# andrewadare/SLAM.jl

Measured on AMD Instinct MI355X. Metric: EKF updates/sec @ 10k landmarks, higher is better.
Workload: dtype f32; 1 GPU; EKF-SLAM observation step (associate+update; no new features arise), N=10000 landmarks (n=20003), nz=64 obs/step, gates 4.0/25.0, cholesky form, state resident in HBM; landmarks=10000, form=cholesky, parallelism=single GPU

## Files before the change

slam.jl_amd/csrc/common.h:

```cpp
#pragma once

#include <hip/hip_runtime.h>
#include <stdint.h>
#include <stdio.h>
#include <string.h>
#include <vector>

#include "../../include/slamhip.h"
#include "../../include/slamhip_diag.h"

#define SLAM_PI 3.14159265358979323846

void slam_set_error(const char* fmt, ...);

#define HIP_TRY(expr)                                                                  \
    do {                                                                               \
        hipError_t _e = (expr);                                                        \
        if (_e != hipSuccess) {                                                        \
            slam_set_error("%s failed: %s (%s:%d)", #expr, hipGetErrorString(_e),     \
                           __FILE__, __LINE__);                                        \
            return (_e == hipErrorOutOfMemory) ? SLAM_E_NOMEM : SLAM_E_HIP;            \
        }                                                                              \
    } while (0)

#define ARG_CHECK(cond, msg)                                                           \
    do {                                                                               \
        if (!(cond)) {                                                                 \
            slam_set_error("bad argument: %s", msg);                                   \
            return SLAM_E_BADARG;                                                      \
        }                                                                              \
    } while (0)

void slam_roctx_push(const char* name);
void slam_roctx_pop(void);
struct SlamRange {
    explicit SlamRange(const char* name) { slam_roctx_push(name); }
    ~SlamRange() { slam_roctx_pop(); }
    SlamRange(const SlamRange&) = delete;
    SlamRange& operator=(const SlamRange&) = delete;
};
#define SLAM_RANGE() SlamRange slam_range_scope_(__func__)

#define SLAM_TILE 128
#define SLAM_KPAD 32

static inline int round_up(int a, int b) { return (a + b - 1) / b * b; }

#ifdef SLAMHIP_EXPERIMENTS
#include <stdlib.h>
static inline int slam_exp_env(const char* name, int dflt) {
    const char* v = getenv(name);
    return v ? atoi(v) : dflt;
}
constexpr int SLAM_XFLAGS_MASK = ~0;
#else
static inline int slam_exp_env(const char*, int dflt) { return dflt; }
constexpr int SLAM_XFLAGS_MASK = 4 | 8 | 16 | 32 | 64 | 128 | 512;
#endif

struct TimingPair {
    hipEvent_t a, b;
    int kid;
};

struct slam_ekf {
    int dtype;
    int device;
    int num_cus;
    int maxN;
    int N;
    int ncap;
    int ld;
    int npad;
    size_t esz;
    void* x;
    void* P;
    void* Pside;
    hipStream_t stream;
    double* PHtS;
    hipEvent_t stage_ev;
    int stage_pending;

    int kcap;
    double* PHt;
    double* Kd;
    void* W1;
    void* W2;
    void* Wimg;
    double* Cmat;
    double* Smat;
    double* Mwork;
    double* gvec;
    double* obsbuf;
    int32_t* idfbuf;
    int ocap;
    double* h_obs;
    int32_t* h_idf;
    int32_t* h_assoc;
    int32_t* d_assoc;
    double* h_obs_dev;
    int32_t* h_assoc_dev;
    double* znbuf;
    int32_t* d_count;
    int32_t* h_flag;
    int32_t* h_flag_dev;
    int32_t obs_seq;

    int2* tiles;
    int tiles_T, tiles_len, tiles_cap;
    int tilesB_off, tilesB_len;
    int tilesH_off, tilesH_len;
    unsigned* dd_claim;
    int tiles_xlen[8];
    int diag_off, diag_len, diag_xlen[8];

    double* d_pmax;
    int pmax_valid;

    int gate_mode;
    int gate_last;
    void* grid_meta;
    int32_t* grid_cells;
    void* grid_items;
    int grid_force;
    int grid_upd;
    int grid_live;
    int grid_n_seen;

    double* gate_part;
    int gate_blocks_cap;

    double* d_small;
    double* h_small;
    int32_t* d_status;
    int32_t* h_status;

    int xflags;
    int debug_flags;
    void* dd_prof;
    int factor_blocked;
    int debug_stamps;
    int async_updates;
    int deferred;
    int pending_status;

    int timing;
    std::vector<TimingPair> pairs;
    std::vector<TimingPair> free_pairs;
    double t_ms[SLAM_K_COUNT];
    double t_sq[SLAM_K_COUNT];
    double t_min[SLAM_K_COUNT];
    int64_t t_n[SLAM_K_COUNT];
};

struct KTimer {
    slam_ekf* h;
    TimingPair p;
    bool on;
    hipStream_t s;
    KTimer(slam_ekf* h_, int kid, hipStream_t stream = nullptr);
    ~KTimer();
};

int launch_ellipses(slam_ekf* h, double* d_out);
int launch_block_gather(slam_ekf* h, int r0, int c0, int nr, int nc, int diag, void* d_out);
int launch_pack(slam_ekf* h, const void* d_src, int lds, int n, int cf, int ncols);
int launch_unpack(slam_ekf* h, void* d_dst, int ldd, int n, int cf, int ncols);
int launch_side_rebuild(slam_ekf* h);
int launch_compact(slam_ekf* h, const int32_t* keep_host, int n_new, int f0);
int launch_find_duplicates(slam_ekf* h, double gate, int32_t* pairs_out, int cap, int* count);
int launch_merge_update(slam_ekf* h, const int32_t* keep, const int32_t* gone, int cnt, const double Rc[4]);
int launch_copy_floor(slam_ekf* h, int reps, double out[2]);
int launch_predict(slam_ekf* h, double v, double g, double w, const double Q[4], double dt);
int launch_augment(slam_ekf* h, int nn, const double R[4], const double* zn_dev);
int launch_gate(slam_ekf* h, int nz, const double R[4], double gate1, double gate2, const double* z_host, bool compact);
constexpr int SLAM_GRID_SLOTS = 64;
int gate_kernels_init();
int gate_info(slam_ekf* h, int64_t out[8]);
unsigned long long* grid_drift_slot(slam_ekf* h);
int ensure_pmax(slam_ekf* h);
int launch_nis(slam_ekf* h, const double z1[2], int j, const double R[4]);
int launch_obs_model(slam_ekf* h, int j);
int launch_update(slam_ekf* h, int m, const double R[4], int form, bool device_count);
int ensure_update_workspace(slam_ekf* h, int m);
int ensure_obs_capacity(slam_ekf* h, int nobs);
```

slam.jl_amd/csrc/ekf_syrk.hip:

```cpp
#include <algorithm>
#include <stdlib.h>

#include "common.h"
#include <type_traits>
#include "device_math.h"

namespace {

typedef float f32x16 __attribute__((ext_vector_type(16)));
typedef float f32x4 __attribute__((ext_vector_type(4)));

constexpr int TILE = SLAM_TILE;
constexpr int KC = 32;
constexpr int LDSP = KC + 4;

__device__ __forceinline__ void wave_lds_fence() {
    __builtin_amdgcn_fence(__ATOMIC_RELEASE, "wavefront");
    __builtin_amdgcn_wave_barrier();
    __builtin_amdgcn_fence(__ATOMIC_ACQUIRE, "wavefront");
}

typedef unsigned u32x4 __attribute__((ext_vector_type(4)));

struct DdCtxP {
// ... 192 lines not shown
    for (int rb = 0; rb < 2; ++rb)
#pragma unroll
        for (int r = 0; r < 16; ++r) {
            const int soff = ((32 * c.wc + 8 * (r >> 2) + (r & 3)) * TILE + 64 * c.wr + 32 * rb) * 4;
            pold[rb][r] = __uint_as_float(__builtin_amdgcn_raw_buffer_load_b32(rs, voff, soff, AUX));
        }
}

template <int AUX = 2>
__device__ __forceinline__ void store_p_mfma(const DdCtx& c, int R0, int C0, const float (&pold)[2][16], f32x16 (&acc)[2]) {
    const auto rs = tile_rsrc(c, R0, C0);
    const int voff = (4 * c.lh * TILE + c.l31) * 4;
    const bool adj = R0 == C0 + TILE;
#pragma unroll
    for (int rb = 0; rb < 2; ++rb)
#pragma unroll
        for (int r = 0; r < 16; ++r) {
            const int soff = ((32 * c.wc + 8 * (r >> 2) + (r & 3)) * TILE + 64 * c.wr + 32 * rb) * 4;
            const float v = pold[rb][r] - acc[rb][r];
            __builtin_amdgcn_raw_buffer_store_b32(__float_as_uint(v), rs, voff, soff, AUX);
            if (rb == 0 && r == 15 && adj && c.wr == 0 && c.wc == 3 && c.lh == 1 && c.l31 == 0) c.side[(size_t)c.side_n + ((C0 + TILE - 4) >> 1)] = v;
            acc[rb][r] = 0.0f;
        }
}

template <int NCH, int POFF = 2>
__device__ __forceinline__ void dd_stream(DdCtx& c, const int2* __restrict__ list, int L, int nper, int& slot, smem_t& smem,
                                          f32x4 (&gx)[2], f32x4 (&gy)[2]) {
    auto fetch = [&](int sl) { return sl < L ? list[sl] : make_int2(-1, -1); };
    constexpr int PCH = NCH - POFF > 0 ? NCH - POFF : 0;
    int2 tile = fetch(slot);
    int2 next = fetch(slot + nper);
    f32x16 acc[2];
#pragma unroll
    for (int rb = 0; rb < 2; ++rb)
#pragma unroll
        for (int r = 0; r < 16; ++r) acc[rb][r] = 0.0f;
    float pold[2][16];
    Frag f0;
    const int last_steps = (c.kp - (NCH - 1) * KC <= 16) ? 2 : 4;
    fill_lds(c, smem, 0, gx, gy);
    __syncthreads();
    request_chunk(c, tile, 1, gx, gy);
    int base = 0;
    for (;;) {
        const bool next_off = next.x >= 0 && next.x != next.y;
#pragma unroll
        for (int ch = 0; ch < NCH; ++ch) {
            const int pb = (base + ch) & 1;
            if (ch == PCH) load_p_mfma(c, tile.x * TILE, tile.y * TILE, pold);
            if (ch < NCH - 1) {
#pragma unroll
                for (int st = 0; st < 4; ++st) {
                    read_frag(c, smem, pb, 8 * st, f0);
                    mfma_step(c, f0, acc);
                }
                fill_lds(c, smem, pb ^ 1, gx, gy);
                __syncthreads();
                if (ch + 2 < NCH) request_chunk(c, tile, ch + 2, gx, gy);
                else if (next.x >= 0) request_chunk(c, next, 0, gx, gy);
            } else {
                for (int st = 0; st < last_steps; ++st) {
                    read_frag(c, smem, pb, 8 * st, f0);
                    mfma_step(c, f0, acc);
                }
                if (next_off) fill_lds(c, smem, pb ^ 1, gx, gy);
                __syncthreads();
                if (next_off) request_chunk(c, next, 1, gx, gy);
                store_p_mfma(c, tile.x * TILE, tile.y * TILE, pold, acc);
            }
        }
        slot += nper;
        if (!next_off) return;
        tile = next;
        next = fetch(slot + nper);
        base = (base + NCH) & 1;
    }
}

typedef __bf16 bf16x8 __attribute__((ext_vector_type(8)));
typedef __bf16 bf16x2 __attribute__((ext_vector_type(2)));
typedef float f32x2 __attribute__((ext_vector_type(2)));
typedef unsigned u32x2 __attribute__((ext_vector_type(2)));
constexpr int KB = 16;
constexpr int BROW = 48;
constexpr int BARR = TILE * BROW;

__device__ __forceinline__ int stage_row(int tid) {
    return (tid >> 6) * 16 + ((tid >> 5) & 1) * 8 + ((tid >> 4) & 1) + 2 * ((tid >> 2) & 3);
}

__device__ __forceinline__ void request_chunk_b(const DdCtx& c, int2 t, int chunk, f32x4& gx, f32x4& gy) {
    const auto rx = __builtin_amdgcn_make_buffer_rsrc(const_cast<float*>(c.X), (short)0, c.ld * c.pitch * 4, 0x00020000);
    const auto ry = __builtin_amdgcn_make_buffer_rsrc(const_cast<float*>(c.Y), (short)0, c.ld * c.pitch * 4, 0x00020000);
    const int tid = threadIdx.x;
    const int voff = (stage_row(tid) * c.pitch + 4 * (tid & 3)) * 4;
    gx = __builtin_bit_cast(f32x4, __builtin_amdgcn_raw_buffer_load_b128(rx, voff, (t.x * TILE * c.pitch + chunk * KB) * 4, 0));
    gy = __builtin_bit_cast(f32x4, __builtin_amdgcn_raw_buffer_load_b128(ry, voff, (t.y * TILE * c.pitch + chunk * KB) * 4, 0));
}

__device__ __forceinline__ void split2(float v0, float v1, unsigned& h, unsigned& m, unsigned& l) {
    const f32x2 v = {v0, v1};
    h = __builtin_bit_cast(unsigned, __builtin_convertvector(v, bf16x2));
    const f32x2 r1 = {v0 - __uint_as_float(h << 16), v1 - __uint_as_float(h & 0xffff0000u)};
    m = __builtin_bit_cast(unsigned, __builtin_convertvector(r1, bf16x2));
    const f32x2 r2 = {r1.x - __uint_as_float(m << 16), r1.y - __uint_as_float(m & 0xffff0000u)};
    l = __builtin_bit_cast(unsigned, __builtin_convertvector(r2, bf16x2));
}

__device__ __forceinline__ void fill_lds_b(const DdCtx& c, char* sm, int buf, const f32x4& gx, const f32x4& gy) {
    const int tid = threadIdx.x;
    char* base = sm + buf * (6 * BARR) + stage_row(tid) * BROW + (tid & 3) * 8;
#pragma unroll
    for (int pnl = 0; pnl < 2; ++pnl) {
        const f32x4 g = pnl ? gy : gx;
        unsigned h0, m0, l0, h1, m1, l1;
        split2(g.x, g.y, h0, m0, l0);
        split2(g.z, g.w, h1, m1, l1);
        *reinterpret_cast<u32x2*>(base + (3 * pnl + 0) * BARR) = u32x2{h0, h1};
        *reinterpret_cast<u32x2*>(base + (3 * pnl + 1) * BARR) = u32x2{m0, m1};
        *reinterpret_cast<u32x2*>(base + (3 * pnl + 2) * BARR) = u32x2{l0, l1};
    }
}

__device__ __forceinline__ void mfma_chunk_b(const DdCtx& c, const char* sm, int buf, f32x16 (&acc)[2]) {
    const char* base = sm + buf * (6 * BARR) + c.l31 * BROW + c.lh * 16;
    bf16x8 a[3];
#pragma unroll
    for (int sp = 0; sp < 3; ++sp) a[sp] = *reinterpret_cast<const bf16x8*>(base + (3 + sp) * BARR + (32 * c.wc) * BROW);
#pragma unroll
    for (int rb = 0; rb < 2; ++rb) {
        bf16x8 b[3];
#pragma unroll
        for (int sp = 0; sp < 3; ++sp) b[sp] = *reinterpret_cast<const bf16x8*>(base + sp * BARR + (64 * c.wr + 32 * rb) * BROW);
        __builtin_amdgcn_s_setprio(3);
        acc[rb] = __builtin_amdgcn_mfma_f32_32x32x16_bf16(a[1], b[1], acc[rb], 0, 0, 0);
        acc[rb] = __builtin_amdgcn_mfma_f32_32x32x16_bf16(a[0], b[2], acc[rb], 0, 0, 0);
        acc[rb] = __builtin_amdgcn_mfma_f32_32x32x16_bf16(a[2], b[0], acc[rb], 0, 0, 0);
        acc[rb] = __builtin_amdgcn_mfma_f32_32x32x16_bf16(a[0], b[1], acc[rb], 0, 0, 0);
        acc[rb] = __builtin_amdgcn_mfma_f32_32x32x16_bf16(a[1], b[0], acc[rb], 0, 0, 0);
        acc[rb] = __builtin_amdgcn_mfma_f32_32x32x16_bf16(a[0], b[0], acc[rb], 0, 0, 0);
        __builtin_amdgcn_s_setprio(0);
    }
}

constexpr int IMG_ARR = TILE * 32;
constexpr int IMG_CHUNK = 3 * IMG_ARR;
typedef unsigned u32x4b __attribute__((ext_vector_type(4)));

__device__ __forceinline__ void request_chunk_p(const DdCtx& c, int2 t, int chunk, u32x4b (&g)[3]) {
    const auto rs = __builtin_amdgcn_make_buffer_rsrc(const_cast<char*>(c.img), (short)0, 0x7fffffff, 0x00020000);
    const int tid = threadIdx.x;
    const int sx = (t.x * c.img_nch + chunk) * IMG_CHUNK, sy = (t.y * c.img_nch + chunk) * IMG_CHUNK;
    g[0] = __builtin_amdgcn_raw_buffer_load_b128(rs, tid * 16, sx, 0);
    g[1] = tid < 256 ? __builtin_amdgcn_raw_buffer_load_b128(rs, (tid + 512) * 16, sx, 0)
                     : __builtin_amdgcn_raw_buffer_load_b128(rs, (tid - 256) * 16, sy, 0);
    g[2] = __builtin_amdgcn_raw_buffer_load_b128(rs, (tid + 256) * 16, sy, 0);
}

__device__ __forceinline__ void fill_lds_p(char* sm, int buf, const u32x4b (&g)[3]) {
    char* base = sm + buf * (2 * IMG_CHUNK) + threadIdx.x * 16;
#pragma unroll
    for (int j = 0; j < 3; ++j) *reinterpret_cast<u32x4b*>(base + j * 8192) = g[j];
}

__device__ __forceinline__ void mfma_chunk_p(const DdCtx& c, const char* sm, int buf, f32x16 (&acc)[2], bool negate = false) {
    const char* base = sm + buf * (2 * IMG_CHUNK) + c.l31 * 32 + ((c.lh ^ (c.l31 >> 3)) & 1) * 16;
    bf16x8 a[3];
#pragma unroll
    for (int sp = 0; sp < 3; ++sp) a[sp] = *reinterpret_cast<const bf16x8*>(base + IMG_CHUNK + sp * IMG_ARR + (32 * c.wc) * 32);
    bf16x8 b[3];
#pragma unroll
    for (int rb = 0; rb < 2; ++rb) {
#pragma unroll
        for (int sp = 0; sp < 3; ++sp) b[sp] = *reinterpret_cast<const bf16x8*>(base + sp * IMG_ARR + (64 * c.wr + 32 * rb) * 32);
        __builtin_amdgcn_s_setprio(3);
        acc[rb] = __builtin_amdgcn_mfma_f32_32x32x16_bf16(a[1], b[1], acc[rb], 0, 0, 0);
        acc[rb] = __builtin_amdgcn_mfma_f32_32x32x16_bf16(a[0], b[2], acc[rb], 0, 0, 0);
        acc[rb] = __builtin_amdgcn_mfma_f32_32x32x16_bf16(a[2], b[0], acc[rb], 0, 0, 0);
        acc[rb] = __builtin_amdgcn_mfma_f32_32x32x16_bf16(a[0], b[1], acc[rb], 0, 0, 0);
        acc[rb] = __builtin_amdgcn_mfma_f32_32x32x16_bf16(a[1], b[0], acc[rb], 0, 0, 0);
        acc[rb] = __builtin_amdgcn_mfma_f32_32x32x16_bf16(a[0], b[0], acc[rb], 0, 0, 0);
        __builtin_amdgcn_s_setprio(0);
    }
}

constexpr int CLAIM_OFF = 2 * 2 * IMG_CHUNK;
typedef __attribute__((address_space(3))) unsigned lds_u32_t;
__device__ __forceinline__ void lds_store_u32(char* p, unsigned v) { *(volatile lds_u32_t*)p = v; }
__device__ __forceinline__ unsigned lds_load_u32(const char* p) { return *(const volatile lds_u32_t*)p; }
#ifndef DD_PCH0
#define DD_PCH0 0
#endif
#ifndef DD_DMA_PCH8
#define DD_DMA_PCH8 2
#endif
#ifndef DD_POFF8
#define DD_POFF8 (7 + DD_PCH0)
#endif

template <int NCH, int POFF, bool WRAP = false, bool DYN = false>
__device__ __forceinline__ void dd_stream_p(DdCtx& c, const int2* __restrict__ list, int L, int nper, int& slot, char* sm,
                                            unsigned* __restrict__ ctr = nullptr) {
    auto fetch = [&](int sl) { return sl < L ? list[sl] : make_int2(-1, -1); };
    auto request_chunk_p = [&](const DdCtx& cc, int2 t, int chunk, u32x4b (&gg)[3]) { ::request_chunk_p(cc, t, WRAP ? (chunk & 7) : chunk, gg); };
    constexpr int PCH = NCH - POFF > 0 ? NCH - POFF : 0;
    static_assert(!DYN || NCH >= 4, "the claimed position is read after chunk 1 and used at chunk NCH - 2");
    int2 tile = fetch(slot);
    int2 next = DYN ? make_int2(-1, -1) : fetch(slot + nper);
    int next_slot = slot + nper;
    unsigned claimed = 0;
    f32x16 acc[2];
#pragma unroll
    for (int rb = 0; rb < 2; ++rb)
#pragma unroll
        for (int r = 0; r < 16; ++r) acc[rb][r] = 0.0f;
    float pold[2][16];
    u32x4b g[3];
    request_chunk_p(c, tile, 0, g);
    fill_lds_p(sm, 0, g);
    __syncthreads();
    request_chunk_p(c, tile, 1, g);
    int base = 0;
    for (;;) {
        bool next_off = next.x >= 0 && next.x != next.y;
#pragma unroll
        for (int ch = 0; ch < NCH; ++ch) {
            const int pb = (base + ch) & 1;
            if (ch == PCH) load_p_mfma(c, tile.x * TILE, tile.y * TILE, pold);
            mfma_chunk_p(c, sm, pb, acc, WRAP && ch >= 8);
            if (DYN && ch == 1 && threadIdx.x == 0) lds_store_u32(sm + CLAIM_OFF, claimed);
            if (ch < NCH - 1) {
                fill_lds_p(sm, pb ^ 1, g);
                __syncthreads();
                if (DYN && ch == 0 && threadIdx.x == 0)
                    claimed = __hip_atomic_fetch_add(ctr, 1u, __ATOMIC_RELAXED, __HIP_MEMORY_SCOPE_AGENT);
                if (DYN && ch == 1) {
                    next_slot = nper + __builtin_amdgcn_readfirstlane((int)lds_load_u32(sm + CLAIM_OFF));
                    next = fetch(next_slot);
                    next_off = next.x >= 0 && next.x != next.y;
                }
                if (ch + 2 < NCH) request_chunk_p(c, tile, ch + 2, g);
                else if (next_off) request_chunk_p(c, next, 0, g);
            } else {
                if (next_off) fill_lds_p(sm, pb ^ 1, g);
                __syncthreads();
                if (next_off) request_chunk_p(c, next, 1, g);
                store_p_mfma(c, tile.x * TILE, tile.y * TILE, pold, acc);
            }
        }
        slot = DYN ? next_slot : slot + nper;
        if (!next_off) return;
        tile = next;
        if (!DYN) next = fetch(slot + nper);
        base = (base + NCH) & 1;
    }
}


constexpr int DMA_BUF = 2 * IMG_CHUNK;
typedef __attribute__((address_space(3))) void lds_void_t;

__device__ __forceinline__ void dma_chunk(const DdCtx& c, int2 t, int chunk, char* sm, int buf, int wave) {
    const auto rs = __builtin_amdgcn_make_buffer_rsrc(const_cast<char*>(c.img), (short)0, 0x7fffffff, 0x00020000);
    const int sx = (t.x * c.img_nch + chunk) * IMG_CHUNK + wave * 1024, sy = (t.y * c.img_nch + chunk) * IMG_CHUNK + wave * 1024;
    const int lane16 = (threadIdx.x & 63) * 16;
    char* dst = sm + buf * DMA_BUF + wave * 1024;
    __builtin_amdgcn_raw_ptr_buffer_load_lds(rs, (lds_void_t*)dst, 16, lane16, sx, 0, 0);
    __builtin_amdgcn_raw_ptr_buffer_load_lds(rs, (lds_void_t*)(dst + 8192), 16, lane16, wave < 4 ? sx + 8192 : sy - 4096, 0, 0);
    __builtin_amdgcn_raw_ptr_buffer_load_lds(rs, (lds_void_t*)(dst + 16384), 16, lane16, sy + 4096, 0, 0);
}
__device__ __forceinline__ unsigned lds_addr(const char* p) { return (unsigned)(unsigned long long)(const lds_void_t*)p; }
__device__ __forceinline__ void asm_lds_store_u32(char* p, unsigned v) {
    asm volatile("ds_write_b32 %0, %1" ::"v"(lds_addr(p)), "v"(v) : "memory");
}
__device__ __forceinline__ unsigned asm_lds_load_u32(const char* p) {
    unsigned v;
    asm volatile("ds_read_b32 %0, %1\n\ts_waitcnt lgkmcnt(0)" : "=v"(v) : "v"(lds_addr(p)) : "memory");
    return v;
}
template <int I, int N, typename F>
__device__ __forceinline__ void static_for(F&& f) {
    if constexpr (I < N) {
        f(std::integral_constant<int, I>{});
        static_for<I + 1, N>(f);
    }
}
template <int N>
__device__ __forceinline__ void wait_vm() { asm volatile("s_waitcnt vmcnt(%0)" ::"n"(N) : "memory"); }
__device__ __forceinline__ void bare_barrier() { asm volatile("s_waitcnt lgkmcnt(0)\n\ts_barrier" ::: "memory"); }

struct DdFrags { bf16x8 a[3], b[3], b1[3]; };
__device__ __forceinline__ void read_frags_d(const DdCtx& c, const char* sm, int buf, DdFrags& f) {
    const unsigned base = lds_addr(sm) + buf * DMA_BUF + c.l31 * 32 + ((c.lh ^ (c.l31 >> 3)) & 1) * 16;
    const unsigned ya = base + IMG_CHUNK + (32 * c.wc) * 32, xa = base + (64 * c.wr) * 32;
    asm volatile(
        "ds_read_b128 %0, %9\n\tds_read_b128 %1, %9 offset:4096\n\tds_read_b128 %2, %9 offset:8192\n\t"
        "ds_read_b128 %3, %10\n\tds_read_b128 %4, %10 offset:4096\n\tds_read_b128 %5, %10 offset:8192\n\t"
        "ds_read_b128 %6, %10 offset:1024\n\tds_read_b128 %7, %10 offset:5120\n\tds_read_b128 %8, %10 offset:9216\n\t"
        "s_waitcnt lgkmcnt(0)"
        : "=&v"(f.a[0]), "=&v"(f.a[1]), "=&v"(f.a[2]), "=&v"(f.b[0]), "=&v"(f.b[1]), "=&v"(f.b[2]), "=&v"(f.b1[0]), "=&v"(f.b1[1]), "=&v"(f.b1[2])
        : "v"(ya), "v"(xa)
        : "memory");
}
__device__ __forceinline__ void mfma_frags_d(const DdFrags& f, f32x16 (&acc)[2]) {
#pragma unroll
    for (int rb = 0; rb < 2; ++rb) {
        __builtin_amdgcn_s_setprio(3);
        acc[rb] = __builtin_amdgcn_mfma_f32_32x32x16_bf16(f.a[1], rb ? f.b1[1] : f.b[1], acc[rb], 0, 0, 0);
        acc[rb] = __builtin_amdgcn_mfma_f32_32x32x16_bf16(f.a[0], rb ? f.b1[2] : f.b[2], acc[rb], 0, 0, 0);
        acc[rb] = __builtin_amdgcn_mfma_f32_32x32x16_bf16(f.a[2], rb ? f.b1[0] : f.b[0], acc[rb], 0, 0, 0);
        acc[rb] = __builtin_amdgcn_mfma_f32_32x32x16_bf16(f.a[0], rb ? f.b1[1] : f.b[1], acc[rb], 0, 0, 0);
        acc[rb] = __builtin_amdgcn_mfma_f32_32x32x16_bf16(f.a[1], rb ? f.b1[0] : f.b[0], acc[rb], 0, 0, 0);
        acc[rb] = __builtin_amdgcn_mfma_f32_32x32x16_bf16(f.a[0], rb ? f.b1[0] : f.b[0], acc[rb], 0, 0, 0);
        __builtin_amdgcn_s_setprio(0);
    }
}

template <int NCH, int PCH>
__device__ __forceinline__ void dd_stream_dma(DdCtx& c, const int2* __restrict__ list, int L, int nper, int& slot, char* sm,
                                              unsigned* __restrict__ ctr, int wave, char* cw) {
    static_assert(NCH >= 5 && PCH >= 2 && PCH <= NCH - 2, "");
    constexpr int RD = NCH - 3;
    auto fetch = [&](int sl) { return sl < L ? list[sl] : make_int2(-1, -1); };
    int2 tile = fetch(slot);
    int2 next = make_int2(-1, -1);
    int next_slot = slot + nper;
    unsigned claimed = 0;
    f32x16 acc[2];
#pragma unroll
    for (int rb = 0; rb < 2; ++rb)
#pragma unroll
        for (int r = 0; r < 16; ++r) acc[rb][r] = 0.0f;
    float pold[2][16];
    dma_chunk(c, tile, 0, sm, 0, wave);
    dma_chunk(c, tile, 1, sm, 1, wave);
    dma_chunk(c, tile, 2, sm, 2, wave);
    wait_vm<6>();
    bare_barrier();
    int base = 0;
    bool first = true;
    for (;;) {
        bool next_off = false;
        static_for<0, NCH>([&](auto CH) {
            constexpr int ch = decltype(CH)::value;
            const int buf = (base + ch) % 3;
            __builtin_amdgcn_sched_barrier(0);
            if (ch == PCH) load_p_mfma(c, tile.x * TILE, tile.y * TILE, pold);
            DdFrags fr;
            read_frags_d(c, sm, buf, fr);
            mfma_frags_d(fr, acc);
            if (ch == RD && threadIdx.x == 0) asm_lds_store_u32(cw, claimed);
            constexpr int PL = (ch == PCH || ch == PCH + 1) ? 32 : 0;
            if (ch <= 1) {
                if (first) wait_vm<3>();
                else wait_vm<35>();
            } else if (ch + 2 < NCH || next_off) wait_vm<3 + PL>();
            else wait_vm<PL>();
            bare_barrier();
            if (ch == 0 && threadIdx.x == 0) claimed = __hip_atomic_fetch_add(ctr, 1u, __ATOMIC_RELAXED, __HIP_MEMORY_SCOPE_AGENT);
            if (ch == RD) {
                next_slot = nper + __builtin_amdgcn_readfirstlane((int)asm_lds_load_u32(cw));
                next = fetch(next_slot);
                next_off = next.x >= 0 && next.x != next.y;
            }
            if (ch + 3 < NCH) dma_chunk(c, tile, ch + 3, sm, buf, wave);
            else if (next_off) dma_chunk(c, next, ch + 3 - NCH, sm, buf, wave);
            __builtin_amdgcn_sched_barrier(0);
            if (ch == NCH - 1) store_p_mfma(c, tile.x * TILE, tile.y * TILE, pold, acc);
        });
        slot = next_slot;
        if (!next_off) break;
        tile = next;
        base = (base + NCH) % 3;
        first = false;
    }
    wait_vm<0>();
}

template <int NCH, int POFF, int AUXL = 2, int AUXS = 2>
__device__ __forceinline__ void dd_stream_b(DdCtx& c, const int2* __restrict__ list, int L, int nper, int& slot, char* sm,
                                            f32x4& gx, f32x4& gy) {
    auto fetch = [&](int sl) { return sl < L ? list[sl] : make_int2(-1, -1); };
    constexpr int PCH = NCH - POFF > 0 ? NCH - POFF : 0;
    int2 tile = fetch(slot);
    int2 next = fetch(slot + nper);
    f32x16 acc[2];
#pragma unroll
    for (int rb = 0; rb < 2; ++rb)
#pragma unroll
        for (int r = 0; r < 16; ++r) acc[rb][r] = 0.0f;
    float pold[2][16];
    fill_lds_b(c, sm, 0, gx, gy);
    __syncthreads();
    request_chunk_b(c, tile, 1, gx, gy);
    int base = 0;
    for (;;) {
        const bool next_off = next.x >= 0 && next.x != next.y;
#pragma unroll
        for (int ch = 0; ch < NCH; ++ch) {
            const int pb = (base + ch) & 1;
            if (ch == PCH) load_p_mfma<AUXL>(c, tile.x * TILE, tile.y * TILE, pold);
            mfma_chunk_b(c, sm, pb, acc);
            if (ch < NCH - 1) {
                fill_lds_b(c, sm, pb ^ 1, gx, gy);
                __syncthreads();
                if (ch + 2 < NCH) request_chunk_b(c, tile, ch + 2, gx, gy);
                else if (next_off) request_chunk_b(c, next, 0, gx, gy);
            } else {
                if (next_off) fill_lds_b(c, sm, pb ^ 1, gx, gy);
                __syncthreads();
                if (next_off) request_chunk_b(c, next, 1, gx, gy);
                store_p_mfma<AUXS>(c, tile.x * TILE, tile.y * TILE, pold, acc);
            }
        }
        slot += nper;
        if (!next_off) return;
        tile = next;
        next = fetch(slot + nper);
        base = (base + NCH) & 1;
    }
}

template <int STREAM = 0, int POFF = 2, bool BF = false>
__global__ __launch_bounds__(NTHREADS) __attribute__((amdgpu_waves_per_eu(4, 4))) void downdate_f32_mfma(float* __restrict__ P, int ld, int n,
                                                                 const float* __restrict__ X, const float* __restrict__ Y,
                                                                 int pitch, int kp, const int2* __restrict__ tiles, int L,
                                                                 const int32_t* __restrict__ status, int xflags,
                                                                 const int32_t* __restrict__ dcount, int joseph,
                                                                 const char* __restrict__ img, int img_nch,
                                                                 unsigned* __restrict__ claim,
                                                                 float* __restrict__ side, int side_n) {
    if (status[0] != 0) return;
    if (dcount) {
        const int k = 2 * dcount[0];
        kp = joseph ? 2 * ((k + SLAM_KPAD - 1) / SLAM_KPAD * SLAM_KPAD) : (k + 15) / 16 * 16;
        if (kp == 0) return;
    }
    __shared__ __attribute__((aligned(16))) float smem[2][2][TILE][LDSP];
    __shared__ unsigned dma_claim_word[4];
    const int tid = threadIdx.x;
    const int lane = tid & 63;
    const int wave = __builtin_amdgcn_readfirstlane(tid >> 6);
    DdCtx c;
    c.side = side; c.side_n = side_n;
    c.P = P; c.X = X; c.Y = Y; c.ld = ld; c.pitch = pitch; c.kp = kp; c.xflags = xflags;
    c.img = img; c.img_nch = img_nch;
    c.nchunks = (kp + KC - 1) / KC;
    c.wr = wave & 1;
    c.wc = wave >> 1;
    c.l31 = lane & 31;
    c.lh = lane >> 5;
    c.q = lane & 7;
    c.cl = lane >> 3;
    c.srow = tid >> 3;
    c.sc4 = tid & 7;
    const int xcd = blockIdx.x & 7;
    const int rk = blockIdx.x >> 3;
    const int nper = gridDim.x >> 3;
    if (nper < L && rk >= (nper >> 1) && !claim) __builtin_amdgcn_s_sleep(127);
    const int2* list = tiles + (size_t)xcd * L;
    float* sD = &smem[0][0][0][0] + wave * (2 * 32 * SP);
    float* sV = sD + 32 * SP;
    (void)n;

    int slot = rk;
    int2 tile = slot < L ? list[slot] : make_int2(-1, -1);
    if (tile.x < 0) return;
    f32x4 gx[2], gy[2];
    if (BF && claim && img && kp >= 5 * KB && kp <= 8 * KB && !joseph) {
        char* sm = reinterpret_cast<char*>(&smem[0][0][0][0]);
        unsigned* ctr = claim + 16 * xcd;
        if (tile.x != tile.y && !(c.xflags & 512)) {
            static_assert(sizeof(smem) == 3 * DMA_BUF, "three 24 KB chunk buffers");
            char* cw = reinterpret_cast<char*>(&dma_claim_word[0]);
            switch (kp / KB) {
                case 8: dd_stream_dma<8, DD_DMA_PCH8>(c, list, L, nper, slot, sm, ctr, wave, cw); break;
                case 7: dd_stream_dma<7, 2>(c, list, L, nper, slot, sm, ctr, wave, cw); break;
                case 6: dd_stream_dma<6, 2>(c, list, L, nper, slot, sm, ctr, wave, cw); break;
                default: dd_stream_dma<5, 2>(c, list, L, nper, slot, sm, ctr, wave, cw); break;
            }
        } else
        if (tile.x != tile.y) {
            switch (kp / KB) {
                case 8: dd_stream_p<8, DD_POFF8, false, true>(c, list, L, nper, slot, sm, ctr); break;
                case 7: dd_stream_p<7, 6 + DD_PCH0, false, true>(c, list, L, nper, slot, sm, ctr); break;
                case 6: dd_stream_p<6, 5 + DD_PCH0, false, true>(c, list, L, nper, slot, sm, ctr); break;
                default: dd_stream_p<5, 4 + DD_PCH0, false, true>(c, list, L, nper, slot, sm, ctr); break;
            }
        }
        while (slot < L) {
            tile = list[slot];
            if (tile.x < 0) break;
            __syncthreads();
            request_chunk(c, tile, 0, gx, gy);
            if (tile.x != tile.y) dd_tile<false>(c, tile, make_int2(-1, -1), smem, sD, sV, gx, gy);
            else dd_tile<true>(c, tile, make_int2(-1, -1), smem, sD, sV, gx, gy);
            if (tid == 0)
                lds_store_u32(sm + CLAIM_OFF, __hip_atomic_fetch_add(ctr, 1u, __ATOMIC_RELAXED, __HIP_MEMORY_SCOPE_AGENT));
            __syncthreads();
            slot = nper + __builtin_amdgcn_readfirstlane((int)lds_load_u32(sm + CLAIM_OFF));
        }
        return;
    }
    if (BF && tile.x != tile.y && kp >= 5 * KB && kp <= 8 * KB && !joseph) {
        char* sm = reinterpret_cast<char*>(&smem[0][0][0][0]);
        if (img) {
            switch (kp / KB) {
                case 8:
                    dd_stream_p<8, 7>(c, list, L, nper, slot, sm); break;
                case 7: dd_stream_p<7, 6>(c, list, L, nper, slot, sm); break;
                case 6: dd_stream_p<6, 5>(c, list, L, nper, slot, sm); break;
                default: dd_stream_p<5, 4>(c, list, L, nper, slot, sm); break;
            }
        } else {
        request_chunk_b(c, tile, 0, gx[0], gy[0]);
        switch (kp / KB) {
            case 8: dd_stream_b<8, 7>(c, list, L, nper, slot, sm, gx[0], gy[0]); break;
            case 7: dd_stream_b<7, 6>(c, list, L, nper, slot, sm, gx[0], gy[0]); break;
            case 6: dd_stream_b<6, 5>(c, list, L, nper, slot, sm, gx[0], gy[0]); break;
            default: dd_stream_b<5, 4>(c, list, L, nper, slot, sm, gx[0], gy[0]); break;
        }
        }
        tile = slot < L ? list[slot] : make_int2(-1, -1);
        if (tile.x < 0) return;
    }
    request_chunk(c, tile, 0, gx, gy);
    slot += nper;
    int2 next = slot < L ? list[slot] : make_int2(-1, -1);
    if (STREAM >= 2 && tile.x != tile.y && c.nchunks == STREAM) {
        slot = rk;
        dd_stream<(STREAM >= 2 ? STREAM : 2), POFF>(c, list, L, nper, slot, smem, gx, gy);
        tile = slot < L ? list[slot] : make_int2(-1, -1);
        slot += nper;
        next = slot < L ? list[slot] : make_int2(-1, -1);
    } else if (tile.x != tile.y) {
        dd_tile<false>(c, tile, next, smem, sD, sV, gx, gy);
        while (next.x >= 0 && next.x != next.y) {
            tile = next;
            slot += nper;
            next = slot < L ? list[slot] : make_int2(-1, -1);
            dd_tile<false>(c, tile, next, smem, sD, sV, gx, gy);
        }
        tile = next;
        slot += nper;
        next = slot < L ? list[slot] : make_int2(-1, -1);
    }
    while (tile.x >= 0) {
        dd_tile<true>(c, tile, next, smem, sD, sV, gx, gy);
        tile = next;
        slot += nper;
        next = slot < L ? list[slot] : make_int2(-1, -1);
    }
}



constexpr int DT = 64;
constexpr int DK = 16;
typedef double f64x4 __attribute__((ext_vector_type(4)));

__global__ __launch_bounds__(256) void downdate_f64_mfma(double* __restrict__ P, int ld, int n, const double* __restrict__ X,
                                                         const double* __restrict__ Y, int pitch, int kp,
                                                         const int2* __restrict__ tiles, int L,
                                                         const int32_t* __restrict__ status,
                                                         const int32_t* __restrict__ dcount, int joseph, int k16,
                                                         double* __restrict__ side, int side_n) {
    if (status[0] != 0) return;
    int khalf = joseph ? kp / 2 : 0;
    if (dcount) {
        const int k = 2 * dcount[0];
        if (k == 0) return;
        k16 = (k + 15) / 16 * 16;
        khalf = joseph ? (k + SLAM_KPAD - 1) / SLAM_KPAD * SLAM_KPAD : 0;
    }
    const int2 tile = tiles[(size_t)(blockIdx.x & 7) * L + (blockIdx.x >> 3)];
    if (tile.x < 0) return;
    __shared__ double sX[DT][DK + 1];
    __shared__ double sY[DT][DK + 1];
    const int tid = threadIdx.x;
    const int lane = tid & 63, wave = tid >> 6;
    const int li = lane & 15, kk = lane >> 4;
    const int wr = wave & 1, wc = wave >> 1;
    const int R0 = tile.x * DT;
    const int C0 = tile.y * DT;
    const bool diag = tile.x == tile.y;
    double* Pt = P + tile_base(tile.x, tile.y, ld >> 6, 6);
    f64x4 pold[2][2], acc[2][2];
    auto load_p = [&]() {
#pragma unroll
        for (int cb = 0; cb < 2; ++cb)
#pragma unroll
            for (int rb = 0; rb < 2; ++rb)
#pragma unroll
                for (int r = 0; r < 4; ++r) {
                    const int cl = 32 * wc + 16 * cb + 4 * r + kk, rl = 32 * wr + 16 * rb + li;
                    pold[cb][rb][r] = Pt[cl * DT + rl];
                }
    };
#pragma unroll
    for (int cb = 0; cb < 2; ++cb)
#pragma unroll
        for (int rb = 0; rb < 2; ++rb) acc[cb][rb] = f64x4{0.0, 0.0, 0.0, 0.0};
    load_p();
    for (int seg = 0; seg <= joseph; ++seg)
    for (int kc = seg * khalf; kc < seg * khalf + k16; kc += DK) {
#pragma unroll
        for (int s = 0; s < 4; ++s) {
            const int idx = tid + 256 * s;
            const int row = idx >> 4;
            const int cc = idx & 15;
            sX[row][cc] = X[(size_t)(R0 + row) * pitch + kc + cc];
            sY[row][cc] = Y[(size_t)(C0 + row) * pitch + kc + cc];
        }
        __syncthreads();
#pragma unroll
        for (int s = 0; s < 4; ++s) {
            double ay[2], bx[2];
#pragma unroll
            for (int cb = 0; cb < 2; ++cb) ay[cb] = sY[32 * wc + 16 * cb + li][4 * s + kk];
#pragma unroll
            for (int rb = 0; rb < 2; ++rb) bx[rb] = sX[32 * wr + 16 * rb + li][4 * s + kk];
#pragma unroll
            for (int cb = 0; cb < 2; ++cb)
#pragma unroll
                for (int rb = 0; rb < 2; ++rb)
                    acc[cb][rb] = __builtin_amdgcn_mfma_f64_16x16x4f64(ay[cb], bx[rb], acc[cb][rb], 0, 0, 0);
        }
        __syncthreads();
    }
#pragma unroll
    for (int cb = 0; cb < 2; ++cb)
#pragma unroll
        for (int rb = 0; rb < 2; ++rb)
#pragma unroll
            for (int r = 0; r < 4; ++r) {
                const int cl = 32 * wc + 16 * cb + 4 * r + kk, rl = 32 * wr + 16 * rb + li;
                const double val = pold[cb][rb][r] - acc[cb][rb][r];
                if (!diag || rl >= cl) Pt[cl * DT + rl] = val;
                if ((diag && rl >= cl) || tile.x == tile.y + 1) side_note(side, side_n, R0 + rl, C0 + cl, val);
                if (diag && rl > cl) Pt[rl * DT + cl] = val;
            }
    (void)n;
}

void build_tile_order(int T, std::vector<int2>& out, int order) {
    constexpr int NX = 8;
    constexpr int SR = 4;
    const int nsr = (T + SR - 1) / SR;
    std::vector<std::vector<int2>> lists(NX);
    if (order == 2) {
        for (int J = 0; J < T; ++J)
            for (int I = J + 1; I < T; ++I) {
                const int r = I % (2 * NX);
                lists[r < NX ? r : 2 * NX - 1 - r].push_back(make_int2(I, J));
            }
    } else {
        std::vector<long> load(NX, 0);
        std::vector<std::vector<int>> mine(NX);
        for (int s = nsr - 1; s >= 0; --s) {
            const int I0 = s * SR, I1 = std::min(T, I0 + SR);
            long cnt = 0;
            for (int I = I0; I < I1; ++I) cnt += I;
            int best = 0;
            for (int xcd = 1; xcd < NX; ++xcd)
                if (load[xcd] < load[best]) best = xcd;
            load[best] += cnt;
            mine[best].push_back(s);
        }
        for (int xcd = 0; xcd < NX; ++xcd)
            for (int s : mine[xcd]) {
                const int I0 = s * SR, I1 = std::min(T, I0 + SR);
                for (int J = 0; J < I1; ++J)
                    for (int I = std::max(I0, J + 1); I < I1; ++I) lists[xcd].push_back(make_int2(I, J));
            }
    }
    for (int I = 0; I < T; ++I) {
        int best = 0;
        for (int xcd = 1; xcd < NX; ++xcd)
            if (lists[xcd].size() < lists[best].size()) best = xcd;
        lists[best].push_back(make_int2(I, I));
    }
    size_t L = 0;
    for (int xcd = 0; xcd < NX; ++xcd) L = std::max(L, lists[xcd].size());
    out.assign(L * NX, make_int2(-1, -1));
    for (int xcd = 0; xcd < NX; ++xcd)
        for (size_t slot = 0; slot < lists[xcd].size(); ++slot) out[xcd * L + slot] = lists[xcd][slot];
}

int ensure_tile_order(slam_ekf* h, int T) {
    if (h->tiles && h->tiles_T == T) return SLAM_OK;
    std::vector<int2> order, orderB, orderH;
    build_tile_order(T, order, 0);
    build_tile_order(T, orderB, 2);
    const size_t total = order.size() + orderB.size() + orderH.size();
    HIP_TRY(hipStreamSynchronize(h->stream));
    if ((int)total > h->tiles_cap) {
        if (h->tiles) (void)hipFree(h->tiles);
        h->tiles = nullptr;
        h->tiles_cap = 0;
        HIP_TRY(hipMalloc((void**)&h->tiles, sizeof(int2) * total));
        h->tiles_cap = (int)total;
    }
    HIP_TRY(hipMemcpy(h->tiles, order.data(), sizeof(int2) * order.size(), hipMemcpyHostToDevice));
    HIP_TRY(hipMemcpy(h->tiles + order.size(), orderB.data(), sizeof(int2) * orderB.size(), hipMemcpyHostToDevice));
    if (!orderH.empty())
        HIP_TRY(hipMemcpy(h->tiles + order.size() + orderB.size(), orderH.data(), sizeof(int2) * orderH.size(), hipMemcpyHostToDevice));
    h->tilesH_off = (int)(order.size() + orderB.size());
    h->tilesH_len = (int)orderH.size() / 8;
    h->tiles_T = T;
    h->tiles_len = (int)order.size() / 8;
    h->tilesB_off = (int)order.size();
    h->tilesB_len = (int)orderB.size() / 8;
    return SLAM_OK;
}

template <typename T>
__global__ __launch_bounds__(512) void tile_copy_floor_kernel(T* __restrict__ P, long long total_bytes, T one) {
    typedef T vec_t __attribute__((ext_vector_type(16 / sizeof(T))));
    const long long nunits = (total_bytes + 65535) >> 16;
    for (long long t = blockIdx.x; t < nunits; t += gridDim.x) {
        char* base = reinterpret_cast<char*>(P) + (t << 16);
        const bool full = (t << 16) + 65536 <= total_bytes;
        vec_t v[8];
#pragma unroll
        for (int u = 0; u < 8; ++u)
            if (full || u < 4) v[u] = __builtin_nontemporal_load(reinterpret_cast<vec_t*>(base) + u * 512 + threadIdx.x);
#pragma unroll
        for (int u = 0; u < 8; ++u)
            if (full || u < 4) __builtin_nontemporal_store(v[u] * one, reinterpret_cast<vec_t*>(base) + u * 512 + threadIdx.x);
    }
}

}


int launch_copy_floor(slam_ekf* h, int reps, double out[2]) {
    const int n = 3 + 2 * h->N;
    const int tlog = h->dtype == SLAM_F32 ? 7 : 6, E = 1 << tlog;
    const long long T = (n + E - 1) / E;
    const long long Tall = h->ld >> tlog;
    const long long ntiles = T * Tall - T * (T - 1) / 2;
    const long long bytes = ntiles * (long long)E * E * (long long)h->esz, units = (bytes + 65535) >> 16;
    auto one_pass = [&](int form) {
        const long long grid = form == 0 ? units : std::min<long long>(units, 2 * h->num_cus);
        if (h->dtype == SLAM_F32)
            hipLaunchKernelGGL(tile_copy_floor_kernel<float>, dim3((unsigned)grid), dim3(512), 0, h->stream, (float*)h->P, bytes, 1.0f);
        else
            hipLaunchKernelGGL(tile_copy_floor_kernel<double>, dim3((unsigned)grid), dim3(512), 0, h->stream, (double*)h->P, bytes, 1.0);
    };
    std::vector<hipEvent_t> ev(reps + 1, nullptr);
    hipError_t e = hipSuccess;
    for (int r = 0; r <= reps && e == hipSuccess; ++r) e = hipEventCreate(&ev[r]);
    double best = 1e30;
    int best_form = 0;
    for (int form = 0; form < 2 && e == hipSuccess; ++form) {
        one_pass(form);
        one_pass(form);
        e = hipEventRecord(ev[0], h->stream);
        for (int r = 0; r < reps && e == hipSuccess; ++r) {
            one_pass(form);
            e = hipEventRecord(ev[r + 1], h->stream);
        }
        if (e == hipSuccess) e = hipGetLastError();
        if (e == hipSuccess) e = hipEventSynchronize(ev[reps]);
        for (int r = 0; r < reps && e == hipSuccess; ++r) {
            float ms = 0.f;
            e = hipEventElapsedTime(&ms, ev[r], ev[r + 1]);
            if (e == hipSuccess && ms < best) { best = ms; best_form = form; }
        }
    }
    for (hipEvent_t x : ev)
        if (x) (void)hipEventDestroy(x);
    if (e != hipSuccess) {
        slam_set_error("HIP error in the copy-floor measurement: %s", hipGetErrorString(e));
        return SLAM_E_HIP;
    }
    out[0] = best;
    out[1] = (double)best_form;
    return SLAM_OK;
}

int launch_downdate(slam_ekf* h, int kp_total, const void* X, const void* Y, int pitch, const int32_t* dcount, int joseph, int k16,
                    const void* img) {
#define IMGARGS (const char*)img, h->kcap / 16, (unsigned*)nullptr, (float*)h->Pside, h->npad / 2
#define IMGARGS_CLAIM (const char*)img, h->kcap / 16, h->dd_claim, (float*)h->Pside, h->npad / 2
    const int n = 3 + 2 * h->N;
    const int edge = h->dtype == SLAM_F32 ? TILE : DT;
    const int rc = ensure_tile_order(h, (n + edge - 1) / edge);
    if (rc) return rc;
    KTimer t(h, SLAM_K_SYRK);
    if (h->dtype == SLAM_F32) {
        int per_xcd = 2 * h->num_cus / 8;
        if (per_xcd > h->tiles_len) per_xcd = h->tiles_len;
        if (per_xcd < 1) per_xcd = 1;
        if (!(h->xflags & 4) && kp_total > 32 && kp_total <= 128) {
            const int nch = (kp_total + KC - 1) / KC;
#define DD_LAUNCH_STREAM4()                                                                                            \
    hipLaunchKernelGGL((downdate_f32_mfma<4, 3>), dim3(8 * per_xcd), dim3(NTHREADS), 0, h->stream, (float*)h->P, h->ld, \
                       n, (const float*)X, (const float*)Y, pitch, kp_total, (const int2*)h->tiles, h->tiles_len,       \
                       h->d_status, h->xflags, dcount, joseph, IMGARGS)
#define DD_LAUNCH_STREAM(NCH)                                                                                          \
    hipLaunchKernelGGL((downdate_f32_mfma<NCH>), dim3(8 * per_xcd), dim3(NTHREADS), 0, h->stream, (float*)h->P, h->ld, \
                       n, (const float*)X, (const float*)Y, pitch, kp_total, (const int2*)h->tiles, h->tiles_len,       \
                       h->d_status, h->xflags, dcount, joseph, IMGARGS)
            if (nch >= 3 && !joseph && !(h->xflags & 8)) {
                const int2* lst = (const int2*)h->tiles + h->tilesB_off;
                const int L = h->tilesB_len;
                const bool dyn = img != nullptr;
                int wgs = dyn ? per_xcd : L;
                if (wgs > L) wgs = L;
                if (wgs < 1) wgs = 1;
                if (dyn) {
                    hipLaunchKernelGGL((downdate_f32_mfma<4, 3, true>), dim3(8 * wgs), dim3(NTHREADS), 0, h->stream,
                                       (float*)h->P, h->ld, n, (const float*)X, (const float*)Y, pitch, kp_total, lst, L,
                                       h->d_status, h->xflags, dcount, joseph, IMGARGS_CLAIM);
                } else
                hipLaunchKernelGGL((downdate_f32_mfma<4, 3, true>), dim3(8 * wgs), dim3(NTHREADS), 0, h->stream,
                                   (float*)h->P, h->ld, n, (const float*)X, (const float*)Y, pitch, kp_total, lst, L,
                                   h->d_status, h->xflags, dcount, joseph, IMGARGS);
            }
            else if (nch == 4) DD_LAUNCH_STREAM4();
            else if (nch == 3) DD_LAUNCH_STREAM(3);
            else DD_LAUNCH_STREAM(2);
#undef DD_LAUNCH_STREAM
#undef DD_LAUNCH_STREAM4
        }
        else
            hipLaunchKernelGGL(downdate_f32_mfma<>, dim3(8 * per_xcd), dim3(NTHREADS), 0, h->stream, (float*)h->P, h->ld, n,
                               (const float*)X, (const float*)Y, pitch, kp_total, (const int2*)h->tiles, h->tiles_len,
                               h->d_status, h->xflags, dcount, joseph, IMGARGS);
    } else {
        const int2* lst = (const int2*)h->tiles;
        const int L = h->tiles_len;
        hipLaunchKernelGGL(downdate_f64_mfma, dim3(8 * L), dim3(256), 0, h->stream, (double*)h->P, h->ld, n,
                           (const double*)X, (const double*)Y, pitch, kp_total, lst, L,
                           h->d_status, dcount, joseph, joseph ? k16 : kp_total, (double*)h->Pside, h->npad / 2);
    }
    HIP_TRY(hipGetLastError());
    return SLAM_OK;
#undef IMGARGS
#undef IMGARGS_CLAIM
}
```

Before: 138,300 obs-updates/s (one observation assimilated = one update).

## Double-buffer LDS fragment reads in streamed DMA downdate kernel

Adds an overlapped variant of the streaming DMA downdate loop. It splits LDS fragment loads into an issue phase and a wait phase and keeps two fragment register sets, so the reads for the next chunk are in flight while MFMAs run on the current one. It also reorders the P tile load and the next-tile DMA prefetch around the final chunks. The new path is the default whenever the dynamic claim image is used, and xflag 65536 turns it off. The cost is higher register pressure and hand-tuned waitcnt values that are fragile to get right.

```diff
diff --git a/slam.jl_amd/csrc/common.h b/slam.jl_amd/csrc/common.h
--- a/slam.jl_amd/csrc/common.h
+++ b/slam.jl_amd/csrc/common.h
@@ -55,7 +55,7 @@
 constexpr int SLAM_XFLAGS_MASK = ~0;
 #else
 static inline int slam_exp_env(const char*, int dflt) { return dflt; }
-constexpr int SLAM_XFLAGS_MASK = 4 | 8 | 16 | 32 | 64 | 128 | 512;
+constexpr int SLAM_XFLAGS_MASK = 4 | 8 | 16 | 32 | 64 | 128 | 512 | 65536;
 #endif
 
 struct TimingPair {
diff --git a/slam.jl_amd/csrc/ekf_syrk.hip b/slam.jl_amd/csrc/ekf_syrk.hip
--- a/slam.jl_amd/csrc/ekf_syrk.hip
+++ b/slam.jl_amd/csrc/ekf_syrk.hip
@@ -518,6 +518,23 @@
         : "=&v"(f.a[0]), "=&v"(f.a[1]), "=&v"(f.a[2]), "=&v"(f.b[0]), "=&v"(f.b[1]), "=&v"(f.b[2]), "=&v"(f.b1[0]), "=&v"(f.b1[1]), "=&v"(f.b1[2])
         : "v"(ya), "v"(xa)
         : "memory");
+}
+__device__ __forceinline__ void issue_frags_d(const DdCtx& c, const char* sm, int buf, DdFrags& f) {
+    const unsigned base = lds_addr(sm) + buf * DMA_BUF + c.l31 * 32 + ((c.lh ^ (c.l31 >> 3)) & 1) * 16;
+    const unsigned ya = base + IMG_CHUNK + (32 * c.wc) * 32, xa = base + (64 * c.wr) * 32;
+    asm volatile(
+        "ds_read_b128 %0, %9\n\tds_read_b128 %1, %9 offset:4096\n\tds_read_b128 %2, %9 offset:8192\n\t"
+        "ds_read_b128 %3, %10\n\tds_read_b128 %4, %10 offset:4096\n\tds_read_b128 %5, %10 offset:8192\n\t"
+        "ds_read_b128 %6, %10 offset:1024\n\tds_read_b128 %7, %10 offset:5120\n\tds_read_b128 %8, %10 offset:9216"
+        : "=&v"(f.a[0]), "=&v"(f.a[1]), "=&v"(f.a[2]), "=&v"(f.b[0]), "=&v"(f.b[1]), "=&v"(f.b[2]), "=&v"(f.b1[0]), "=&v"(f.b1[1]), "=&v"(f.b1[2])
+        : "v"(ya), "v"(xa)
+        : "memory");
+}
+__device__ __forceinline__ void wait_frags_d(DdFrags& f) {
+    asm volatile("s_waitcnt lgkmcnt(0)"
+                 : "+v"(f.a[0]), "+v"(f.a[1]), "+v"(f.a[2]), "+v"(f.b[0]), "+v"(f.b[1]), "+v"(f.b[2]), "+v"(f.b1[0]), "+v"(f.b1[1]), "+v"(f.b1[2])
+                 :
+                 : "memory");
 }
 __device__ __forceinline__ void mfma_frags_d(const DdFrags& f, f32x16 (&acc)[2]) {
 #pragma unroll
@@ -594,6 +611,93 @@
     wait_vm<0>();
 }
 
+template <int NCH>
+__device__ __forceinline__ void dd_stream_dma_ovl(DdCtx& c, const int2* __restrict__ list, int L, int nper, int& slot, char* sm,
+                                                  unsigned* __restrict__ ctr, int wave, char* cw) {
+    static_assert(NCH >= 5, "");
+    constexpr int RD = NCH - 3;
+    auto fetch = [&](int sl) { return sl < L ? list[sl] : make_int2(-1, -1); };
+    int2 tile = fetch(slot);
+    int2 next = make_int2(-1, -1);
+    int next_slot = slot + nper;
+    unsigned claimed = 0;
+    f32x16 acc[2];
+#pragma unroll
+    for (int rb = 0; rb < 2; ++rb)
+#pragma unroll
+        for (int r = 0; r < 16; ++r) acc[rb][r] = 0.0f;
+    dma_chunk(c, tile, 0, sm, 0, wave);
+    dma_chunk(c, tile, 1, sm, 1, wave);
+    dma_chunk(c, tile, 2, sm, 2, wave);
+    wait_vm<6>();
+    bare_barrier();
+    int base = 0;
+    bool first = true;
+    for (;;) {
+        bool next_off = false;
+        DdFrags fr[2];
+        asm volatile("" : "+s"(base));
+        __builtin_amdgcn_sched_barrier(0);
+        issue_frags_d(c, sm, base, fr[0]);
+        static_for<0, NCH - 2>([&](auto CH) {
+            constexpr int ch = decltype(CH)::value;
+            const int buf = (base + ch) % 3;
+            __builtin_amdgcn_sched_barrier(0);
+            if (ch == RD && threadIdx.x == 0) asm_lds_store_u32(cw, claimed);
+            if (ch <= 1) {
+                if (first) wait_vm<3>();
+                else wait_vm<35>();
+            } else wait_vm<3>();
+            wait_frags_d(fr[ch & 1]);
+            bare_barrier();
+            issue_frags_d(c, sm, (base + ch + 1) % 3, fr[(ch + 1) & 1]);
+            if (ch == 0 && threadIdx.x == 0) claimed = __hip_atomic_fetch_add(ctr, 1u, __ATOMIC_RELAXED, __HIP_MEMORY_SCOPE_AGENT);
+            if (ch == RD) {
+                next_slot = nper + __builtin_amdgcn_readfirstlane((int)asm_lds_load_u32(cw));
+                next = fetch(next_slot);
+                next_off = next.x >= 0 && next.x != next.y;
+            }
+            if (ch + 3 < NCH) dma_chunk(c, tile, ch + 3, sm, buf, wave);
+            else if (next_off) dma_chunk(c, next, ch + 3 - NCH, sm, buf, wave);
+            __builtin_amdgcn_sched_barrier(0);
+            mfma_frags_d(fr[ch & 1], acc);
+        });
+        {
+            constexpr int ch = NCH - 2;
+            float pold[2][16];
+            __builtin_amdgcn_sched_barrier(0);
+            DdCtx cp = c;
+            unsigned lane;
+            asm volatile("v_mbcnt_lo_u32_b32 %0, -1, 0\n\tv_mbcnt_hi_u32_b32 %0, -1, %0" : "=v"(lane));
+            cp.l31 = lane & 31;
+            cp.lh = lane >> 5;
+            load_p_mfma(cp, tile.x * TILE, tile.y * TILE, pold);
+            __builtin_amdgcn_sched_barrier(0);
+            wait_frags_d(fr[ch & 1]);
+            mfma_frags_d(fr[ch & 1], acc);
+            if (next_off) wait_vm<35>();
+            else wait_vm<32>();
+            bare_barrier();
+            if (next_off) dma_chunk(c, next, 1, sm, (base + ch) % 3, wave);
+            __builtin_amdgcn_sched_barrier(0);
+            read_frags_d(c, sm, (base + ch + 1) % 3, fr[(ch + 1) & 1]);
+            mfma_frags_d(fr[(ch + 1) & 1], acc);
+            if (next_off) wait_vm<35>();
+            else wait_vm<0>();
+            bare_barrier();
+            if (next_off) dma_chunk(c, next, 2, sm, (base + ch + 1) % 3, wave);
+            __builtin_amdgcn_sched_barrier(0);
+            store_p_mfma(cp, tile.x * TILE, tile.y * TILE, pold, acc);
+        }
+        slot = next_slot;
+        if (!next_off) break;
+        tile = next;
+        base = (base + NCH) % 3;
+        first = false;
+    }
+    wait_vm<0>();
+}
+
 template <int NCH, int POFF, int AUXL = 2, int AUXS = 2>
 __device__ __forceinline__ void dd_stream_b(DdCtx& c, const int2* __restrict__ list, int L, int nper, int& slot, char* sm,
                                             f32x4& gx, f32x4& gy) {
@@ -638,7 +742,7 @@
     }
 }
 
-template <int STREAM = 0, int POFF = 2, bool BF = false>
+template <int STREAM = 0, int POFF = 2, bool BF = false, bool OVL = false>
 __global__ __launch_bounds__(NTHREADS) __attribute__((amdgpu_waves_per_eu(4, 4))) void downdate_f32_mfma(float* __restrict__ P, int ld, int n,
                                                                  const float* __restrict__ X, const float* __restrict__ Y,
                                                                  int pitch, int kp, const int2* __restrict__ tiles, int L,
@@ -690,7 +794,13 @@
         if (tile.x != tile.y && !(c.xflags & 512)) {
             static_assert(sizeof(smem) == 3 * DMA_BUF, "three 24 KB chunk buffers");
             char* cw = reinterpret_cast<char*>(&dma_claim_word[0]);
-            switch (kp / KB) {
+            if constexpr (OVL) switch (kp / KB) {
+                case 8: dd_stream_dma_ovl<8>(c, list, L, nper, slot, sm, ctr, wave, cw); break;
+                case 7: dd_stream_dma_ovl<7>(c, list, L, nper, slot, sm, ctr, wave, cw); break;
+                case 6: dd_stream_dma_ovl<6>(c, list, L, nper, slot, sm, ctr, wave, cw); break;
+                default: dd_stream_dma_ovl<5>(c, list, L, nper, slot, sm, ctr, wave, cw); break;
+            }
+            else switch (kp / KB) {
                 case 8: dd_stream_dma<8, DD_DMA_PCH8>(c, list, L, nper, slot, sm, ctr, wave, cw); break;
                 case 7: dd_stream_dma<7, 2>(c, list, L, nper, slot, sm, ctr, wave, cw); break;
                 case 6: dd_stream_dma<6, 2>(c, list, L, nper, slot, sm, ctr, wave, cw); break;
@@ -1027,7 +1137,11 @@
                 int wgs = dyn ? per_xcd : L;
                 if (wgs > L) wgs = L;
                 if (wgs < 1) wgs = 1;
-                if (dyn) {
+                if (dyn && !(h->xflags & 65536)) {
+                    hipLaunchKernelGGL((downdate_f32_mfma<4, 3, true, true>), dim3(8 * wgs), dim3(NTHREADS), 0, h->stream,
+                                       (float*)h->P, h->ld, n, (const float*)X, (const float*)Y, pitch, kp_total, lst, L,
+                                       h->d_status, h->xflags, dcount, joseph, IMGARGS_CLAIM);
+                } else if (dyn) {
                     hipLaunchKernelGGL((downdate_f32_mfma<4, 3, true>), dim3(8 * wgs), dim3(NTHREADS), 0, h->stream,
                                        (float*)h->P, h->ld, n, (const float*)X, (const float*)Y, pitch, kp_total, lst, L,
                                        h->d_status, h->xflags, dcount, joseph, IMGARGS_CLAIM);
```

New measurement: 145,800 obs-updates/s (one observation assimilated = one update), median of 6. 1.05x the previous value.
